# wkh923/m3pc

Measured on AMD Instinct MI355X. Metric: MPC plan-steps/sec (N=1024, H=16, hopper-medium-v2); independent plan steps, 3 in flight, higher is better.
Workload: dtype bf16; 1 GPU; hopper-medium-v2 shapes (S=11,A=3) rtg_guiding N=1024 H=16 T=32 bf16 candidate pass + fp32 policy pass + fp32 re-score (arg-max and multinomial draw certified under the calibrated bound delta, 8.4 candidates re-scored on average); 3 independent plan steps in flight (policy pass / candidate pass / re-score of neighbouring steps on different streams); window resident in HBM; candidates_per_gpu=1024, global_candidates=1024, horizon=16, traj_length=32, steps_in_flight=3, settle_steps=24, parallelism=1 GPU

## Files before the change

include/m3pc_hip_debug.h:

```cpp
#ifndef M3PC_HIP_DEBUG_H
#define M3PC_HIP_DEBUG_H

#ifdef __cplusplus
extern "C" {
#endif

int m3pc_debug_gemm(int dtype, const void* A, const void* Wt, const float* bias, const float* res, void* C, int M, int N,
                    int K, int gelu, int f32out, int variant, void* stream);
typedef struct m3pc_debug_gemm_args {
    int dtype;
    const void* A;
    int lda;
    int amap[3];
    const void* W;
    int ldw;
    int M, N, K;
    const float* bias;
    const float* rowtab;
    int rt_mod, rt_ld;
    int gelu;
    const float* res;
    int ldr;
    void* C;
    int f32out;
    int ldc;
    int cmap[3];
    float* ws;
    long long ws_bytes;
    int a_padded;
    const float* ln_g;
    const float* ln_b;
    float* ln_out;
    const float* a_ln_g;
    const float* a_ln_b;
    int variant;
    void* stream;
    int* picked;
} m3pc_debug_gemm_args;
int m3pc_debug_gemm_ex(const m3pc_debug_gemm_args* a);
int m3pc_debug_gemm_plan(const m3pc_debug_gemm_args* a);
int m3pc_debug_gemm_group(const m3pc_debug_gemm_args* a, int n);
int m3pc_debug_clock(long long* out2);
int m3pc_debug_clock_big(long long* out4);
int m3pc_debug_topk(const float* v, int n, int k, int* idx_out, void* stream);
int m3pc_debug_calibrate_stats(const float* scores_low, const float* f32, int n, float factor, float* stats, float* delta_out,
                               void* stream);
int m3pc_debug_topk_race_batch(const float* scores, const float* expo, float temperature, int n_windows, int n_total, int kmax, int kmin,
                               int rmax, int* list, float* list_scores, void* stream);
int m3pc_debug_gather_listed(const float* sample_actions, const int* list, int n_windows, int n_total, int row_floats, int list_stride,
                             int lo, int hi, float* cand, int* window_index, void* stream);
typedef struct m3pc_debug_tail_args {
    const float* scores;
    const float* expo;
    int race, select;
    float temperature;
    int n_windows, n_total;
    const int* list;
    const float* list_scores;
    const float* list_rescored;
    int rmax, list_stride, f_stride, f_lo;
    const int* r;
    const int* n;
    const float* delta;
    float* merged;
    float* stats;
    float* host_stats;
    float seq;
    const float* a0;
    long long a0_window_stride, a0_stride;
    int A;
    float* p;
    float* eval_action;
    int* argmax;
    int* sample_idx;
    float* sample_action;
    void* stream;
} m3pc_debug_tail_args;
int m3pc_debug_merge_select_batch(const m3pc_debug_tail_args* a);
int m3pc_debug_select_batch(const float* scores, const float* a0, long long a0_window_stride, long long a0_stride, int n_windows,
                            int n_total, int A, float temperature, const float* expo, float* p, float* eval_action, int* argmax,
                            int* sample_idx, float* sample_action, void* stream);
typedef struct m3pc_debug_eval_batch_args {
    const float* merged;
    int n_windows, n_total;
    const int* list;
    int rmax, list_stride, n_listed;
    const int* r;
    const int* n;
// ... 147 lines not shown
```

m3pc_amd/build.py:

```python
from __future__ import annotations

import os
import subprocess
import sys
from concurrent.futures import ThreadPoolExecutor

HERE = os.path.dirname(os.path.abspath(__file__))
CSRC = os.path.join(HERE, "csrc")
LIB = os.path.join(HERE, "libm3pc_hip.so")
SOURCES = ["gemm.hip", "gemm_x3.hip", "gemm_glds.hip", "gemm_big.hip", "gemm_line.hip", "gemm_f32_direct.hip", "block_fused.hip", "attn.hip",
           "attn_bf16.hip", "elementwise.hip", "select.hip", "refine.hip", "m3pc_plans.hip", "m3pc_passes.hip", "m3pc.hip", "m3pc_certified.hip"]
LAB_SOURCES = ["gemm_ring.hip", "gemm_persist.hip", "gemm_rs.hip", "m3pc_debug.hip"]
LAB_LIB = os.path.join(HERE, "libm3pc_hip_lab.so")
ARCH = "gfx950"
EXTRA_FLAGS = {"block_fused.hip": ["-fno-slp-vectorize"]}


def _hipcc() -> str:
    for c in (os.environ.get("HIPCC"), "/opt/rocm/bin/hipcc", "hipcc"):
        if c and (os.path.isabs(c) and os.path.exists(c) or not os.path.isabs(c)):
            return c
    raise RuntimeError("hipcc not found")


def _stale(target: str, deps) -> bool:
    if not os.path.exists(target):
        return True
    t = os.path.getmtime(target)
    return any(os.path.getmtime(d) > t for d in deps)


def build_library(force: bool = False, verbose: bool = False, lab: bool = False) -> str:
    hipcc = _hipcc()
    headers = [os.path.join(CSRC, n) for n in ("kernels.h", "gemm_epilogue.h", "gemm_stage_asm.h", "m3pc_internal.h", "cert_resolve.h", "exports.map")] + \
              [os.path.join(os.path.dirname(HERE), "include", n) for n in ("m3pc_hip.h", "m3pc_hip_debug.h")]
    objdir = os.path.join(CSRC, "build_lab" if lab else "build")
    os.makedirs(objdir, exist_ok=True)
    flags = ["-O3", f"--offload-arch={ARCH}", "-fPIC", "-std=c++17", "-Wall", "-Wno-unused-function",
             "-fno-gpu-rdc", "-ffp-contract=off", "-fvisibility=hidden"] + (["-DM3PC_LAB"] if lab else [])
    jobs = []
    objs = []
    lib = LAB_LIB if lab else LIB
    for s in SOURCES + (LAB_SOURCES if lab else []):
        src = os.path.join(CSRC, s)
        obj = os.path.join(objdir, s.replace(".hip", ".o"))
        objs.append(obj)
        if force or _stale(obj, [src] + headers):
            jobs.append([hipcc, *flags, *EXTRA_FLAGS.get(s, []), "-c", src, "-o", obj])

    def run(cmd):
        if verbose:
            print(" ".join(cmd), flush=True)
        r = subprocess.run(cmd, capture_output=True, text=True)
        if r.returncode != 0:
            raise RuntimeError("hipcc failed:\n" + " ".join(cmd) + "\n" + r.stdout + r.stderr)
        if verbose and r.stderr.strip():
            print(r.stderr)

    with ThreadPoolExecutor(max_workers=4) as ex:
        list(ex.map(run, jobs))
    if force or jobs or _stale(lib, objs):
        run([hipcc, "-shared", "-fPIC", f"--offload-arch={ARCH}", f"-Wl,--version-script={os.path.join(CSRC, 'exports.map')}", "-o", lib, *objs])
    return lib


if __name__ == "__main__":
    print(build_library(force="--force" in sys.argv, verbose=True, lab="--lab" in sys.argv))
```

m3pc_amd/csrc/gemm.hip:

```cpp
#include "kernels.h"

namespace m3pc {

#ifdef M3PC_LAB
thread_local int g_gemm_picked[4] = {0, 0, 0, 0};
thread_local int g_gemm_dry = 0;
#endif

typedef float f32x16 __attribute__((ext_vector_type(16)));
typedef float f32x4 __attribute__((ext_vector_type(4)));
typedef __bf16 bf16x8 __attribute__((ext_vector_type(8)));
typedef unsigned int u32x4 __attribute__((ext_vector_type(4)));

#define LDS_ROW 144

enum { EPI_GELU = 1, EPI_RES = 2, EPI_ROWTAB = 4, EPI_F32OUT = 8, EPI_SPLITK = 16 };

__device__ __forceinline__ float gelu_exact(float x) { return 0.5f * x * (1.0f + erff(x * 0.70710678118654752440f)); }
__device__ __forceinline__ float gelu_fast(float x) {
    const float ax = fabsf(x) * 0.70710678118654752440f;
    const float t = __builtin_amdgcn_rcpf(fmaf(0.3275911f, ax, 1.0f));
    float p = fmaf(t, 1.061405429f, -1.453152027f);
    p = fmaf(t, p, 1.421413741f);
    p = fmaf(t, p, -0.284496736f);
    p = fmaf(t, p, 0.254829592f);
    p *= t;
    const float e = __builtin_amdgcn_exp2f(-ax * ax * 1.44269504088896340736f);
    const float erf_abs = fmaf(-p, e, 1.0f);
    const float hx = 0.5f * x;
    return fmaf(fabsf(hx), erf_abs, hx);
}

__device__ __forceinline__ int map_row(const RowMap& m, int r) {
    if (m.rpg == 0) return r;
    return (r / m.rpg) * m.gstride + (r % m.rpg) + m.off;
}

template <typename T, int BM, int BN, int EPI>
__global__ __launch_bounds__(256) void gemm_kernel(GemmP p) {
    constexpr int TM = BM / 64, TN = BN / 64;
    constexpr int A_CH = BM * 8 / 256, W_CH = BN * 8 / 256;
    constexpr int BUF = (BM + BN) * LDS_ROW;
    __shared__ __attribute__((aligned(16))) char smem[2 * BUF];

    const int tid = threadIdx.x;
    const int lane = tid & 63, wid = tid >> 6;
    const int wr = wid >> 1, wc = wid & 1;
    const int ntn = p.N / BN;
    const int ntm = (p.M + BM - 1) / BM;
    const int nwg = ntm * ntn;
    int bid = blockIdx.x;
    {
        const int q = nwg / 8, r = nwg % 8, x = bid % 8, i = bid / 8;
        bid = (x < r ? x * (q + 1) : r * (q + 1) + (x - r) * q) + i;
    }
    const int tm = bid / ntn, tn = bid % ntn;
    const int row0 = tm * BM, col0 = tn * BN;

    const char* Ab = (const char*)p.A;
    const char* Wb = (const char*)p.W;
    const long long lda_b = (long long)p.lda * sizeof(T), ldw_b = (long long)p.ldw * sizeof(T);
    const int nkt = (int)((long long)p.K * sizeof(T) / 128);
    int kt0 = 0, kt1 = nkt;
    if constexpr (EPI & EPI_SPLITK) {
        kt0 = (int)((long long)nkt * blockIdx.y / gridDim.y);
        kt1 = (int)((long long)nkt * (blockIdx.y + 1) / gridDim.y);
    }

    const char* a_src[A_CH];
    int a_dst[A_CH];
#pragma unroll
    for (int i = 0; i < A_CH; ++i) {
        const int c = tid + i * 256, r = c >> 3, kc = c & 7;
        int gr = row0 + r;
        if (gr >= p.M) gr = p.M - 1;
        a_src[i] = Ab + (long long)map_row(p.amap, gr) * lda_b + kc * 16 + (long long)kt0 * 128;
        a_dst[i] = r * LDS_ROW + kc * 16;
    }
    const char* w_src[W_CH];
    int w_dst[W_CH];
#pragma unroll
    for (int i = 0; i < W_CH; ++i) {
        const int c = tid + i * 256, r = c >> 3, kc = c & 7;
        w_src[i] = Wb + (long long)(col0 + r) * ldw_b + kc * 16 + (long long)kt0 * 128;
        w_dst[i] = BM * LDS_ROW + r * LDS_ROW + kc * 16;
    }

    f32x16 acc[TM][TN];
#pragma unroll
    for (int i = 0; i < TM; ++i)
#pragma unroll
        for (int j = 0; j < TN; ++j)
#pragma unroll
            for (int e = 0; e < 16; ++e) acc[i][j][e] = 0.f;

    const int nloc = kt1 - kt0;
    u32x4 ra0[A_CH], rw0[W_CH], ra1[A_CH], rw1[W_CH];
    auto gload = [&](u32x4* ra, u32x4* rw, int kt) {
        const long long ko = (long long)kt * 128;
#pragma unroll
        for (int i = 0; i < A_CH; ++i) ra[i] = *(const u32x4*)(a_src[i] + ko);
#pragma unroll
        for (int i = 0; i < W_CH; ++i) rw[i] = *(const u32x4*)(w_src[i] + ko);
    };
    auto lstore = [&](const u32x4* ra, const u32x4* rw, char* buf) {
#pragma unroll
        for (int i = 0; i < A_CH; ++i) *(u32x4*)(buf + a_dst[i]) = ra[i];
#pragma unroll
        for (int i = 0; i < W_CH; ++i) *(u32x4*)(buf + w_dst[i]) = rw[i];
    };
    gload(ra0, rw0, 0);
    lstore(ra0, rw0, smem);
    if (nloc > 1) gload(ra0, rw0, 1);
    if (nloc > 2) gload(ra1, rw1, 2);
    __syncthreads();

    const int fragA = (wr * (BM / 2) + (lane & 31)) * LDS_ROW + 16 * (lane >> 5);
    const int fragW = BM * LDS_ROW + (wc * (BN / 2) + (lane & 31)) * LDS_ROW + 16 * (lane >> 5);

    auto compute = [&](const char* cur) {
#pragma unroll
        for (int s = 0; s < 4; ++s) {
            u32x4 fa[TM], fw[TN];
#pragma unroll
            for (int i = 0; i < TM; ++i) fa[i] = *(const u32x4*)(cur + fragA + i * 32 * LDS_ROW + 32 * s);
#pragma unroll
            for (int j = 0; j < TN; ++j) fw[j] = *(const u32x4*)(cur + fragW + j * 32 * LDS_ROW + 32 * s);
#pragma unroll
            for (int i = 0; i < TM; ++i)
#pragma unroll
                for (int j = 0; j < TN; ++j) {
                    if constexpr (sizeof(T) == 2) {
                        acc[i][j] = __builtin_amdgcn_mfma_f32_32x32x16_bf16(
                            __builtin_bit_cast(bf16x8, fa[i]), __builtin_bit_cast(bf16x8, fw[j]), acc[i][j], 0, 0, 0);
                    } else {
                        const f32x4 a4 = __builtin_bit_cast(f32x4, fa[i]);
                        const f32x4 w4 = __builtin_bit_cast(f32x4, fw[j]);
#pragma unroll
                        for (int e = 0; e < 4; ++e)
                            acc[i][j] = __builtin_amdgcn_mfma_f32_32x32x2f32(a4[e], w4[e], acc[i][j], 0, 0, 0);
                    }
                }
        }
    };
    auto step = [&](u32x4* ra, u32x4* rw, int kt) {
        compute(smem + (kt & 1) * BUF);
        if (kt + 1 < nloc) lstore(ra, rw, smem + ((kt + 1) & 1) * BUF);
        __syncthreads();
        if (kt + 3 < nloc) gload(ra, rw, kt + 3);
    };
    for (int kt = 0; kt < nloc; kt += 2) {
        step(ra0, rw0, kt);
        if (kt + 1 < nloc) step(ra1, rw1, kt + 1);
    }

    if constexpr (EPI & EPI_SPLITK) {
        float* slab = p.ws + (long long)blockIdx.y * p.M * p.N;
#pragma unroll
        for (int i = 0; i < TM; ++i)
#pragma unroll
            for (int reg = 0; reg < 16; ++reg) {
                const int r = row0 + wr * (BM / 2) + i * 32 + (reg & 3) + 8 * (reg >> 2) + 4 * (lane >> 5);
                if (r < p.M) {
#pragma unroll
                    for (int j = 0; j < TN; ++j)
                        slab[(long long)r * p.N + col0 + wc * (BN / 2) + j * 32 + (lane & 31)] = acc[i][j][reg];
                }
            }
        return;
    }
    float bj[TN];
#pragma unroll
    for (int j = 0; j < TN; ++j) bj[j] = p.bias ? p.bias[col0 + wc * (BN / 2) + j * 32 + (lane & 31)] : 0.f;
#pragma unroll
    for (int i = 0; i < TM; ++i) {
#pragma unroll
        for (int reg = 0; reg < 16; ++reg) {
            const int r = row0 + wr * (BM / 2) + i * 32 + (reg & 3) + 8 * (reg >> 2) + 4 * (lane >> 5);
            if (r < p.M) {
                const long long pr = map_row(p.cmap, r);
#pragma unroll
                for (int j = 0; j < TN; ++j) {
                    const int c = col0 + wc * (BN / 2) + j * 32 + (lane & 31);
                    float v = acc[i][j][reg] + bj[j];
                    if constexpr (EPI & EPI_ROWTAB) v += p.rowtab[(long long)(r % p.rt_mod) * p.rt_ld + c];
                    if constexpr (EPI & EPI_GELU) v = sizeof(T) == 2 ? gelu_fast(v) : gelu_exact(v);
                    if constexpr (EPI & EPI_RES) v += p.res[pr * p.ldr + c];
                    if constexpr ((EPI & EPI_F32OUT) || sizeof(T) == 4)
                        p.Cf[pr * p.ldc + c] = v;
                    else
                        p.Cb[pr * p.ldc + c] = (bf16_t)v;
                }
            }
        }
    }
}

__global__ __launch_bounds__(256) void splitk_reduce_kernel(GemmP p, int S, int exact_gelu) {
    const long long n = (long long)p.M * p.N;
    for (long long x = blockIdx.x * 256LL + threadIdx.x; x < n; x += (long long)gridDim.x * 256) {
        const int r = (int)(x / p.N), c = (int)(x % p.N);
        float v = 0.f;
        for (int s = 0; s < S; ++s) v += p.ws[(long long)s * n + x];
        if (p.bias) v += p.bias[c];
        if (p.rowtab) v += p.rowtab[(long long)(r % p.rt_mod) * p.rt_ld + c];
        if (p.gelu) v = exact_gelu ? gelu_exact(v) : gelu_fast(v);
        const long long pr = map_row(p.cmap, r);
        if (p.res) v += p.res[pr * p.ldr + c];
        if (p.Cf) p.Cf[pr * p.ldc + c] = v;
        if (p.Cb) p.Cb[pr * p.ldc + c] = (bf16_t)v;
// ... 32 lines not shown
            for (; k < S; ++k) a += *(const f32x4r*)(src + k * mn);
#pragma unroll
            for (int e = 0; e < 4; ++e) {
                float x = a[e];
                if (p.bias) x += p.bias[c + e];
                if (p.rowtab) x += p.rowtab[(long long)(r % p.rt_mod) * p.rt_ld + c + e];
                if (p.gelu) x = exact_gelu ? gelu_exact(x) : gelu_fast(x);
                if (p.res) x += p.res[(long long)r * p.ldr + c + e];
                a[e] = x;
            }
            *(f32x4r*)(p.Cf + (long long)r * p.ldc + c) = a;
            v[i] = a;
            s += (a[0] + a[1]) + (a[2] + a[3]);
        }
    const float inv_d = 1.0f / (float)p.N;
    const float mean = wave_sum_r(s) * inv_d;
    float q = 0.f;
#pragma unroll
    for (int i = 0; i < 4; ++i)
        if (i < n) {
#pragma unroll
            for (int e = 0; e < 4; ++e) {
                const float c = v[i][e] - mean;
                q += c * c;
            }
        }
    const float rstd = rsqrtf(wave_sum_r(q) * inv_d + 1e-5f);
#pragma unroll
    for (int i = 0; i < 4; ++i)
        if (i < n) {
            const int c = i * 256 + lane * 4;
            const f32x4r g = *(const f32x4r*)(p.ln_g + c);
            const f32x4r b = *(const f32x4r*)(p.ln_b + c);
            f32x4r y;
#pragma unroll
            for (int e = 0; e < 4; ++e) y[e] = (v[i][e] - mean) * rstd * g[e] + b[e];
            *(f32x4r*)(p.ln_out + (long long)r * p.N + c) = y;
        }
}

int launch_splitk_reduce(const GemmP& p, int S, int exact_gelu, hipStream_t st) {
    if (p.ln_g && p.ln_out && p.Cf && !p.Cb && p.cmap.rpg == 0 && p.N % 256 == 0 && p.N <= 1024 && p.ldc % 4 == 0 &&
        (!p.res || p.ldr % 4 == 0)) {
        M3PC_GEMM_LAUNCH(splitk_reduce_ln_kernel, dim3((p.M + 3) / 4), dim3(256), 0, st, p, S, exact_gelu);
        M3PC_GEMM_PICK_FLAG(2);
        return 1;
    }
    const long long n = (long long)p.M * p.N;
    const int g = (int)((n + 255) / 256 < 1024 ? (n + 255) / 256 : 1024);
    M3PC_GEMM_LAUNCH(splitk_reduce_kernel, dim3(g), dim3(256), 0, st, p, S, exact_gelu);
    return 0;
}

template <typename T, int BM, int BN, int EPI>
static void launch_cfg(const GemmP& p, hipStream_t st) {
    const int grid = ((p.M + BM - 1) / BM) * (p.N / BN);
    M3PC_GEMM_LAUNCH((gemm_kernel<T, BM, BN, EPI>), dim3(grid), dim3(256), 0, st, p);
}

template <typename T, int EPI>
static int launch_epi(const GemmP& p, hipStream_t st) {
    const long long big_tiles = (long long)((p.M + 127) / 128) * (p.N / 128);
    if ((p.N % 128) != 0 || big_tiles < 512) {
        const long long tiles = (long long)((p.M + 63) / 64) * (p.N / 64);
        const int nkt = (int)((long long)p.K * sizeof(T) / 128);
        int S = 1;
        if (sizeof(T) == 4 && p.ws && tiles < 768 && (tiles < 200 || nkt > 16)) {
            S = (int)((1023 + tiles) / tiles);
            if (S > nkt / 4) S = nkt / 4;
            if (S > 16) S = 16;
            while (S > 1 && (long long)S * p.M * p.N * 4 > p.ws_bytes) --S;
        }
        M3PC_GEMM_PICK(sizeof(T) == 4 ? 1 : 3, S, 0, 0);
        if (S > 1) {
            M3PC_GEMM_LAUNCH((gemm_kernel<T, 64, 64, EPI_SPLITK>), dim3((unsigned)tiles, S), dim3(256), 0, st, p);
            return launch_splitk_reduce(p, S, (int)(sizeof(T) == 4), st);
        } else {
            launch_cfg<T, 64, 64, EPI>(p, st);
        }
    } else {
        M3PC_GEMM_PICK(sizeof(T) == 4 ? 2 : 4, 1, 0, 0);
        launch_cfg<T, 128, 128, EPI>(p, st);
    }
    return 0;
}

template <typename T>
static int launch_t(const GemmP& p, hipStream_t st) {
    const bool f32out = sizeof(T) == 4 || p.Cf != nullptr;
    const int epi = (p.gelu ? EPI_GELU : 0) | (p.res ? EPI_RES : 0) | (p.rowtab ? EPI_ROWTAB : 0) |
                    (f32out && sizeof(T) == 2 ? EPI_F32OUT : 0);
    switch (epi) {
        case 0: return launch_epi<T, 0>(p, st);
        case EPI_F32OUT: return launch_epi<T, EPI_F32OUT>(p, st);
        case EPI_GELU: return launch_epi<T, EPI_GELU>(p, st);
        case EPI_GELU | EPI_F32OUT: return launch_epi<T, EPI_GELU | EPI_F32OUT>(p, st);
        case EPI_RES: return launch_epi<T, EPI_RES>(p, st);
        case EPI_RES | EPI_F32OUT: return launch_epi<T, EPI_RES | EPI_F32OUT>(p, st);
        case EPI_ROWTAB: return launch_epi<T, EPI_ROWTAB>(p, st);
        case EPI_ROWTAB | EPI_F32OUT: return launch_epi<T, EPI_ROWTAB | EPI_F32OUT>(p, st);
        default: M3PC_GEMM_PICK(0, 0, 0, 0); return 0;
    }
}

int launch_gemm(const GemmP& p, int dtype, hipStream_t st) {
    if (p.M <= 0) return 0;
#ifdef M3PC_LAB
    if (dtype == DT_BF16 && p.variant == 9 && launch_gemm_persist(p, st)) return 0;
    if (dtype == DT_BF16 && p.variant == 36 && launch_gemm_rs(p, st)) return 0;
#endif
    static const bool no_big = M3PC_ENV("M3PC_NO_GEMM_BIG") != nullptr;
    if (dtype == DT_BF16 && p.variant >= 37 && p.variant <= 42 && launch_gemm_big(p, st)) return 0;
    if (dtype == DT_BF16 && p.variant >= 43 && p.variant <= 46 && launch_gemm_line(p, p.variant == 44 ? 256 : 128, st)) return 0;
    static const bool no_line = M3PC_ENV("M3PC_NO_GEMM_LINE") != nullptr;
    static const long long line_min = M3PC_ENV("M3PC_LINE_MIN_TILES") ? atoll(M3PC_ENV("M3PC_LINE_MIN_TILES")) : 256;
    if (dtype == DT_BF16 && p.variant == 0 && !no_line && !p.res && p.K < 1024 &&
        (long long)((p.M + 127) / 128) * (p.N / 128) >= line_min && launch_gemm_line(p, 128, st))
        return 0;
    if (dtype == DT_BF16 && p.variant == 0 && !no_big && p.K >= 1024 && (long long)((p.M + 255) / 256) * (p.N / 256) >= 224 &&
        launch_gemm_big(p, st))
        return 0;
#ifdef M3PC_LAB
    if (dtype == DT_BF16 && p.variant >= 7 && p.variant != 9 && p.variant < 20 && launch_gemm_ring(p, st)) return 0;
#endif
    if (dtype == DT_BF16 && (p.variant == 0 || (p.variant >= 2 && p.variant < 7) || (p.variant >= 20 && p.variant <= 32)) &&
        launch_gemm_glds(p, st))
        return 0;
    if (dtype == DT_BF16) return launch_t<bf16_t>(p, st);
    static const bool no_direct = M3PC_ENV("M3PC_NO_F32_DIRECT") != nullptr;
    if (p.ws && p.variant != 2 && !no_direct && launch_gemm_f32_direct(p, st)) return 0;
    return launch_t<float>(p, st);
}

}
```

m3pc_amd/csrc/gemm_x3.hip:

```cpp
#include "gemm_epilogue.h"

namespace m3pc {

typedef float x3_f32x16 __attribute__((ext_vector_type(16)));
typedef float x3_f32x4 __attribute__((ext_vector_type(4)));
typedef __bf16 x3_bf16x8 __attribute__((ext_vector_type(8)));
typedef __bf16 x3_bf16x4 __attribute__((ext_vector_type(4)));
typedef unsigned int x3_u32x4 __attribute__((ext_vector_type(4)));
typedef unsigned int x3_u32x2 __attribute__((ext_vector_type(2)));

#define X3_ROW 144
enum { X3_SPLITK = 1 << 8 };

__device__ __forceinline__ void x3_split4(x3_u32x4 raw, x3_u32x2& hi, x3_u32x2& lo) {
    const x3_f32x4 x = __builtin_bit_cast(x3_f32x4, raw);
    x3_bf16x4 h, l;
#pragma unroll
    for (int e = 0; e < 4; ++e) {
        h[e] = (__bf16)x[e];
        l[e] = (__bf16)(x[e] - (float)h[e]);
    }
    hi = __builtin_bit_cast(x3_u32x2, h);
    lo = __builtin_bit_cast(x3_u32x2, l);
}

__device__ __forceinline__ int x3_map_row(const RowMap& m, int r) {
    if (m.rpg == 0) return r;
    return (r / m.rpg) * m.gstride + (r % m.rpg) + m.off;
}

template <int BM, int BN, int EPI>
__global__ __launch_bounds__(256) void gemm_x3_kernel(GemmP p) {
    constexpr int TM = BM / 64, TN = BN / 64;
    constexpr int A_CH = BM * 8 / 256, W_CH = BN * 8 / 256;
    constexpr int BUF = (BM + BN) * X3_ROW;
    __shared__ __attribute__((aligned(16))) char smem[2 * BUF];

    const int tid = threadIdx.x;
    const int lane = tid & 63, wid = tid >> 6;
    const int wr = wid >> 1, wc = wid & 1;
    const int ntn = p.N / BN;
    const int ntm = (p.M + BM - 1) / BM;
    const int nwg = ntm * ntn;
    int bid = blockIdx.x;
    {
        const int q = nwg / 8, r = nwg % 8, x = bid % 8, i = bid / 8;
        bid = (x < r ? x * (q + 1) : r * (q + 1) + (x - r) * q) + i;
    }
    const int tm = bid / ntn, tn = bid % ntn;
    const int row0 = tm * BM, col0 = tn * BN;

    const char* Ab = (const char*)p.A;
    const char* Wb = (const char*)p.W;
    const long long lda_b = (long long)p.lda * 4, ldw_b = (long long)p.ldw * 2, wlo_b = p.w_lo_off * 2;
    const int nkt = p.K / 32;
    int kt0 = 0, kt1 = nkt;
    if constexpr (EPI & X3_SPLITK) {
        kt0 = (int)((long long)nkt * blockIdx.y / gridDim.y);
        kt1 = (int)((long long)nkt * (blockIdx.y + 1) / gridDim.y);
    }

    const char* a_src[A_CH];
    int a_dst[A_CH];
#pragma unroll
    for (int i = 0; i < A_CH; ++i) {
        const int c = tid + i * 256, r = c >> 3, kc = c & 7;
        int gr = row0 + r;
        if (gr >= p.M) gr = p.M - 1;
        a_src[i] = Ab + (long long)x3_map_row(p.amap, gr) * lda_b + kc * 16 + (long long)kt0 * 128;
        a_dst[i] = r * X3_ROW + kc * 8;
    }
    const char* w_src[W_CH];
    int w_dst[W_CH];
#pragma unroll
    for (int i = 0; i < W_CH; ++i) {
        const int c = tid + i * 256, r = c >> 3, kc = c & 7;
        w_src[i] = Wb + (long long)(col0 + r) * ldw_b + (kc & 3) * 16 + (kc >> 2) * wlo_b + (long long)kt0 * 64;
        w_dst[i] = BM * X3_ROW + r * X3_ROW + kc * 16;
    }

    x3_f32x16 acc[TM][TN];
#pragma unroll
    for (int i = 0; i < TM; ++i)
#pragma unroll
        for (int j = 0; j < TN; ++j)
#pragma unroll
            for (int e = 0; e < 16; ++e) acc[i][j][e] = 0.f;

    const int nloc = kt1 - kt0;
    x3_u32x4 ra0[A_CH], rw0[W_CH], ra1[A_CH], rw1[W_CH];
    auto gload = [&](x3_u32x4* ra, x3_u32x4* rw, int kt) {
#pragma unroll
        for (int i = 0; i < A_CH; ++i) ra[i] = *(const x3_u32x4*)(a_src[i] + (long long)kt * 128);
#pragma unroll
        for (int i = 0; i < W_CH; ++i) rw[i] = *(const x3_u32x4*)(w_src[i] + (long long)kt * 64);
    };
    auto lstore = [&](const x3_u32x4* ra, const x3_u32x4* rw, char* buf) {
#pragma unroll
        for (int i = 0; i < A_CH; ++i) {
            x3_u32x2 hi, lo;
            x3_split4(ra[i], hi, lo);
            *(x3_u32x2*)(buf + a_dst[i]) = hi;
            *(x3_u32x2*)(buf + a_dst[i] + 64) = lo;
        }
#pragma unroll
        for (int i = 0; i < W_CH; ++i) *(x3_u32x4*)(buf + w_dst[i]) = rw[i];
    };
    gload(ra0, rw0, 0);
    lstore(ra0, rw0, smem);
    if (nloc > 1) gload(ra0, rw0, 1);
    if (nloc > 2) gload(ra1, rw1, 2);
    __syncthreads();

    const int fragA = (wr * (BM / 2) + (lane & 31)) * X3_ROW + 16 * (lane >> 5);
    const int fragW = BM * X3_ROW + (wc * (BN / 2) + (lane & 31)) * X3_ROW + 16 * (lane >> 5);

    auto compute = [&](const char* cur) {
#pragma unroll
        for (int s = 0; s < 2; ++s) {
            x3_u32x4 ah[TM], al[TM], wh[TN], wl[TN];
#pragma unroll
            for (int i = 0; i < TM; ++i) {
                ah[i] = *(const x3_u32x4*)(cur + fragA + i * 32 * X3_ROW + 32 * s);
                al[i] = *(const x3_u32x4*)(cur + fragA + i * 32 * X3_ROW + 64 + 32 * s);
            }
#pragma unroll
            for (int j = 0; j < TN; ++j) {
                wh[j] = *(const x3_u32x4*)(cur + fragW + j * 32 * X3_ROW + 32 * s);
                wl[j] = *(const x3_u32x4*)(cur + fragW + j * 32 * X3_ROW + 64 + 32 * s);
            }
#pragma unroll
            for (int i = 0; i < TM; ++i)
#pragma unroll
                for (int j = 0; j < TN; ++j) {
                    const x3_bf16x8 a_h = __builtin_bit_cast(x3_bf16x8, ah[i]), a_l = __builtin_bit_cast(x3_bf16x8, al[i]);
                    const x3_bf16x8 w_h = __builtin_bit_cast(x3_bf16x8, wh[j]), w_l = __builtin_bit_cast(x3_bf16x8, wl[j]);
                    acc[i][j] = __builtin_amdgcn_mfma_f32_32x32x16_bf16(a_h, w_h, acc[i][j], 0, 0, 0);
                    acc[i][j] = __builtin_amdgcn_mfma_f32_32x32x16_bf16(a_h, w_l, acc[i][j], 0, 0, 0);
                    acc[i][j] = __builtin_amdgcn_mfma_f32_32x32x16_bf16(a_l, w_h, acc[i][j], 0, 0, 0);
                }
        }
    };
    auto step = [&](x3_u32x4* ra, x3_u32x4* rw, int kt) {
        compute(smem + (kt & 1) * BUF);
        if (kt + 1 < nloc) lstore(ra, rw, smem + ((kt + 1) & 1) * BUF);
        __syncthreads();
        if (kt + 3 < nloc) gload(ra, rw, kt + 3);
    };
    for (int kt = 0; kt < nloc; kt += 2) {
        step(ra0, rw0, kt);
        if (kt + 1 < nloc) step(ra1, rw1, kt + 1);
    }

    if constexpr (EPI & X3_SPLITK) {
        float* slab = p.ws + (long long)blockIdx.y * p.M * p.N;
#pragma unroll
        for (int i = 0; i < TM; ++i)
#pragma unroll
            for (int reg = 0; reg < 16; ++reg) {
                const int r = row0 + wr * (BM / 2) + i * 32 + (reg & 3) + 8 * (reg >> 2) + 4 * (lane >> 5);
                if (r < p.M) {
#pragma unroll
                    for (int j = 0; j < TN; ++j)
                        slab[(long long)r * p.N + col0 + wc * (BN / 2) + j * 32 + (lane & 31)] = acc[i][j][reg];
                }
            }
        return;
    } else {
        const int wu = __builtin_amdgcn_readfirstlane(wid);
        const int rbase = row0 + (wu >> 1) * (BM / 2), cbase = col0 + (wu & 1) * (BN / 2);
        gemm_epilogue<EPI, TM, TN>(p, acc, rbase, cbase, row0, BM, lane);
    }
}

__global__ __launch_bounds__(256) void f32_split_bf16_kernel(const float* in, bf16_t* hi, bf16_t* lo, long long n) {
    for (long long x = blockIdx.x * 256LL + threadIdx.x; x < n; x += (long long)gridDim.x * 256) {
        const float v = in[x];
        const bf16_t b = (bf16_t)v;
        hi[x] = b;
        lo[x] = (bf16_t)(v - (float)b);
    }
}
void launch_f32_split_bf16(const float* in, bf16_t* hi, bf16_t* lo, long long n, hipStream_t st) {
    if (n <= 0) return;
    const long long g = (n + 255) / 256;
    hipLaunchKernelGGL(f32_split_bf16_kernel, dim3((unsigned)(g < 4096 ? g : 4096)), dim3(256), 0, st, in, hi, lo, n);
}

template <int BM, int BN, int EPI>
static void x3_launch(const GemmP& p, int S, hipStream_t st) {
    const int grid = ((p.M + BM - 1) / BM) * (p.N / BN);
    M3PC_GEMM_LAUNCH((gemm_x3_kernel<BM, BN, EPI>), dim3(grid, S), dim3(256), 0, st, p);
}

template <int EPI>
static int x3_launch_epi(const GemmP& p, hipStream_t st) {
    const long long big_tiles = (long long)((p.M + 127) / 128) * (p.N / 128);
    if ((p.N % 128) == 0 && big_tiles >= 512) {
        M3PC_GEMM_PICK(13, 1, 0, 0);
        x3_launch<128, 128, EPI>(p, 1, st);
        return 0;
    }
    const long long tiles = (long long)((p.M + 63) / 64) * (p.N / 64);
    const int nkt = p.K / 32;
    int S = 1;
    if (p.ws && tiles < 768 && (tiles < 200 || nkt > 16)) {
        S = (int)((1023 + tiles) / tiles);
        if (S > nkt / 4) S = nkt / 4;
        if (S > 16) S = 16;
        while (S > 1 && (long long)S * p.M * p.N * 4 > p.ws_bytes) --S;
    }
    M3PC_GEMM_PICK(12, S, 0, 0);
    if (S > 1) {
        x3_launch<64, 64, X3_SPLITK>(p, S, st);
        return launch_splitk_reduce(p, S, 1, st);
    }
    x3_launch<64, 64, EPI>(p, 1, st);
    return 0;
}

int launch_gemm_x3(const GemmP& p, hipStream_t st) {
    if (p.M <= 0) return 0;
    if (p.K % 32 != 0 || p.N % 64 != 0 || p.w_lo_off <= 0 || p.w_lo_off % 8 != 0 || (p.Cf == nullptr) == (p.Cb == nullptr)) return -1;
    if (((uintptr_t)p.A & 15) || ((uintptr_t)p.W & 15) || p.lda % 4 != 0 || p.ldw % 8 != 0 || p.a_ln_g) return -1;
    const int epi = (p.gelu ? GE_GELU | GE_GELU_EXACT : 0) | (p.res ? GE_RES : 0) | (p.rowtab ? GE_ROWTAB : 0) |
                    (p.Cf ? GE_F32OUT : 0);
    switch (epi) {
        case GE_F32OUT: return x3_launch_epi<GE_F32OUT>(p, st);
        case GE_GELU | GE_GELU_EXACT | GE_F32OUT: return x3_launch_epi<GE_GELU | GE_GELU_EXACT | GE_F32OUT>(p, st);
        case GE_RES | GE_F32OUT: return x3_launch_epi<GE_RES | GE_F32OUT>(p, st);
        case GE_ROWTAB | GE_F32OUT: return x3_launch_epi<GE_ROWTAB | GE_F32OUT>(p, st);
        case 0: return x3_launch_epi<0>(p, st);
        case GE_GELU | GE_GELU_EXACT: return x3_launch_epi<GE_GELU | GE_GELU_EXACT>(p, st);
        default: return -1;
    }
}

}
```

m3pc_amd/csrc/kernels.h:

```cpp
#pragma once
#include <hip/hip_runtime.h>
#include <stdint.h>

#ifdef M3PC_LAB
#define M3PC_ENV(name) getenv(name)
#else
#define M3PC_ENV(name) ((const char*)nullptr)
#endif

namespace m3pc {

typedef __bf16 bf16_t;

enum DType { DT_F32 = 0, DT_BF16 = 1, DT_X3 = 2 };

static inline size_t dtype_size(int dt) { return dt == DT_F32 ? 4 : 2; }

#ifndef M3PC_STREAM_AUX
#define M3PC_STREAM_AUX 0
#endif
template <typename V>
__device__ __forceinline__ V stream_load(const V* p) { return M3PC_STREAM_AUX ? __builtin_nontemporal_load(p) : *p; }
template <typename V>
__device__ __forceinline__ void stream_store(V v, V* p) {
    if (M3PC_STREAM_AUX) __builtin_nontemporal_store(v, p);
    else *p = v;
}

struct RowMap {
    int rpg;
    int gstride;
    int off;
};
static inline RowMap rowmap_identity() { return RowMap{0, 0, 0}; }

struct GemmP {
    const void* A;
    int lda;
    RowMap amap;
    const void* W;
    int ldw;
    int M, N, K;
    const float* bias;
    const float* rowtab;
    int rt_mod, rt_ld;
    int gelu;
    const float* res;
    int ldr;
    float* Cf;
    bf16_t* Cb;
    int ldc;
    RowMap cmap;
    float* ws;
    long long ws_bytes;
    int a_padded;
    int variant;
    int peel;
    const float* ln_g;
    const float* ln_b;
    float* ln_out;
    const float* a_ln_g;
    const float* a_ln_b;
    long long w_lo_off;
};
struct HeadFusedP {
    const float* X;
    int ldx;
    int rows, d;
    int n_heads;
    int grp, row_mod;
    const float *gA, *bA;
    const float *gB[2], *bB[2];
    const float *W1[2], *b1[2];
    const float *w2[2], *b2[2];
    const float *mean[2], *stdv[2];
    float* out[2];
    float* part;
    int* ticket;
};
bool launch_head_f32_fused(const HeadFusedP& p, hipStream_t st);
int launch_gemm(const GemmP& p, int dtype, hipStream_t st);
int launch_gemm_x3(const GemmP& p, hipStream_t st);
void launch_f32_split_bf16(const float* in, bf16_t* hi, bf16_t* lo, long long n, hipStream_t st);
int launch_splitk_reduce(const GemmP& p, int S, int exact_gelu, hipStream_t st);
bool gemm_f32_direct_covers(const GemmP& p);
bool launch_gemm_f32_direct_group(const GemmP* ps, int n, hipStream_t st);
bool launch_gemm_ring(const GemmP& p, hipStream_t st);
bool launch_gemm_persist(const GemmP& p, hipStream_t st);
bool launch_gemm_rs(const GemmP& p, hipStream_t st);
bool launch_gemm_big(const GemmP& p, hipStream_t st);
bool launch_gemm_line(const GemmP& p, int bt, hipStream_t st);
bool launch_gemm_glds(const GemmP& p, hipStream_t st);
void read_big_probe(long long out[4]);
void read_clock_probe(long long out[2]);
bool launch_gemm_f32_direct(const GemmP& p, hipStream_t st);

__host__ __device__ inline int block_res_row_xb(int r, int L, int nshared) {
    const int b = r / L, w = r % L;
    return w < nshared ? w : nshared + b * (L - nshared) + (w - nshared);
}

struct BlockP {
    const bf16_t* O;
    int ldo;
    int M;
    const float* res;
    int ldr;
    int res_L, res_nshared;
    const float* rowtab;
    int rt_mod;
    int res_nu;
    const bf16_t* wstream;
    const float* bo;
    const float* b1;
    const float* b2;
    const float* ln2_g;
    const float* ln2_b;
    float* Xout;
    int ldx;
    int x_bf16;
    const float* lnA_g;
    const float* lnA_b;
    const float* lnB_g[2];
    const float* lnB_b[2];
    int out_mod, out_grp;
    bf16_t* Hout;
    int ldh;
    bf16_t* QKVout;
    int ldq;
    unsigned qkv_bytes;
    const float* bqkv;
    float* head_out[2];
    const float* hb1[2];
    const float* hw2[2];
    const float* hb2[2];
    const float* hmean[2];
    const float* hstd[2];
    int split;
    int variant;
    long long* stamps;
    int stamp_block;
};
bool block_fused_supported(int d, int ff);
size_t block_stream_bytes();
void launch_pack_block_stream(const bf16_t* Wo, const bf16_t* W1, const bf16_t* W2, bf16_t* out, hipStream_t st);
void launch_pack_block_qkv(const bf16_t* Wqkv_next, bf16_t* out, hipStream_t st);
void launch_pack_block_heads(const bf16_t* Wh0, const bf16_t* Wh1, bf16_t* out, hipStream_t st);
bool launch_block_fused(const BlockP& p, hipStream_t st);
// ... 349 lines not shown
```

m3pc_amd/csrc/m3pc_debug.hip:

```cpp
#include "m3pc_internal.h"

#pragma GCC visibility push(default)
extern "C" {

int m3pc_debug_step_streams_created(m3pc_handle* h) { return h ? h->step_streams_created : -1; }
int m3pc_debug_gemm(int dtype, const void* A, const void* Wt, const float* bias, const float* res, void* C, int M, int N,
                    int K, int gelu, int f32out, int variant, void* stream) {
    static const int ldpad = M3PC_ENV("M3PC_DEBUG_LDPAD") ? atoi(M3PC_ENV("M3PC_DEBUG_LDPAD")) : 0;
    GemmP p = gemm_basic(A, K + ldpad, Wt, K + ldpad, M, N, K, bias);
    p.a_padded = 0;
    p.gelu = gelu;
    p.res = res;
    p.ldr = N;
    p.variant = variant;
    if (dtype == DT_BF16 && !f32out)
        p.Cb = (bf16_t*)C;
    else
        p.Cf = (float*)C;
    p.ldc = N;
    if (dtype != DT_BF16 && variant != 1) {
        static float* ws = nullptr;
        if (!ws) HIPCHK(hipMalloc((void**)&ws, 64 << 20));
        p.ws = ws;
        p.ws_bytes = 64 << 20;
    }
    if (dtype == DT_X3) {
        static bf16_t* wsplit = nullptr;
        static size_t cap = 0;
        const size_t n = (size_t)N * (K + ldpad);
        if (n > cap) {
            if (wsplit) HIPCHK(hipFree(wsplit));
            wsplit = nullptr;
            cap = 0;
            HIPCHK(hipMalloc((void**)&wsplit, 2 * n * sizeof(bf16_t)));
            cap = n;
        }
        launch_f32_split_bf16((const float*)Wt, wsplit, wsplit + n, (long long)n, (hipStream_t)stream);
        p.W = wsplit;
        p.w_lo_off = (long long)n;
        if (launch_gemm_x3(p, (hipStream_t)stream) < 0) return fail(M3PC_EINVAL, "debug_gemm: shape not covered by the x3 kernel");
        return check_launch("debug_gemm");
    }
    launch_gemm(p, dtype, (hipStream_t)stream);
    return check_launch("debug_gemm");
}

static int debug_gemm_fill(const m3pc_debug_gemm_args* a, GemmP& p) {
    if (!a) return fail(M3PC_EINVAL, "debug_gemm_ex: null argument");
    const int dt = a->dtype;
    if (dt != DT_F32 && dt != DT_BF16 && dt != DT_X3) return fail(M3PC_EINVAL, "debug_gemm_ex: dtype %d", dt);
    if (!a->A || !a->W || !a->C) return fail(M3PC_EINVAL, "debug_gemm_ex: null operand");
    if (a->M < 1 || a->M > (1 << 20) || a->N < 32 || a->N > (1 << 16) || a->K < 1 || a->K > (1 << 16)) return fail(M3PC_EINVAL, "debug_gemm_ex: M / N / K out of range");
    const int es = dt == DT_BF16 ? 2 : 4;
    if (a->N % 32) return fail(M3PC_EINVAL, "debug_gemm_ex: N %d is not a multiple of 32 (columns would be dropped)", a->N);
    if (((long long)a->K * es) % 128) return fail(M3PC_EINVAL, "debug_gemm_ex: K %d is not a whole number of 128-byte k-tiles (k terms would be dropped)", a->K);
    if (dt == DT_F32 && !a->f32out) return fail(M3PC_EINVAL, "debug_gemm_ex: fp32 operands have fp32 output only");
    const int f32out = dt == DT_F32 || a->f32out;
    const int os = f32out ? 4 : 2;
    const uintptr_t ptrs = (uintptr_t)a->A | (uintptr_t)a->W | (uintptr_t)a->C | (uintptr_t)a->bias | (uintptr_t)a->rowtab | (uintptr_t)a->res |
                           (uintptr_t)a->ws | (uintptr_t)a->ln_g | (uintptr_t)a->ln_b | (uintptr_t)a->ln_out | (uintptr_t)a->a_ln_g |
                           (uintptr_t)a->a_ln_b;
    if (ptrs & 15) return fail(M3PC_EINVAL, "debug_gemm_ex: pointers must be 16-byte aligned");
    if (a->lda < a->K || a->ldw < a->K || a->ldc < a->N || (a->res && a->ldr < a->N) || (a->rowtab && a->rt_ld < a->N))
        return fail(M3PC_EINVAL, "debug_gemm_ex: a leading dimension is below its row length");
    if (((long long)a->lda * es) % 16 || ((long long)a->ldw * (dt == DT_F32 ? 4 : 2)) % 16 || (dt == DT_X3 && a->ldw % 4) || ((long long)a->ldc * os) % 16 ||
        (a->res && a->ldr % 4) || (a->rowtab && a->rt_ld % 4))
        return fail(M3PC_EINVAL, "debug_gemm_ex: rows of a leading dimension leave 16-byte alignment");
    if (a->rowtab && a->rt_mod < 1) return fail(M3PC_EINVAL, "debug_gemm_ex: rowtab with rt_mod %d", a->rt_mod);
    for (const int* m : {a->amap, a->cmap})
        if (m[0] < 0 || m[2] < 0 || (m[0] >= 1 && m[1] < m[0])) return fail(M3PC_EINVAL, "debug_gemm_ex: row map {%d, %d, %d}", m[0], m[1], m[2]);
    if (a->ws && a->ws_bytes < 0) return fail(M3PC_EINVAL, "debug_gemm_ex: negative ws_bytes");
    if (a->ln_out && (!f32out || !a->ln_g || !a->ln_b)) return fail(M3PC_EINVAL, "debug_gemm_ex: ln_out needs fp32 C, ln_g and ln_b");
    if ((a->a_ln_g != nullptr) != (a->a_ln_b != nullptr)) return fail(M3PC_EINVAL, "debug_gemm_ex: a_ln_g and a_ln_b go together");
    const int v = a->variant;
    if (!(v == 0 || (dt == DT_BF16 && (v == 2 || v == 26 || v == 37 || v == 43 || v == 44)) || (dt == DT_F32 && v == 2)))
        return fail(M3PC_EINVAL, "debug_gemm_ex: variant %d of dtype %d is not one this hook drives", v, dt);
    if (v == 44 && a->a_padded && a->M % 256 && 256 - a->M % 256 > 127)
        return fail(M3PC_EINVAL, "debug_gemm_ex: variant 44 with a_padded would read %d rows behind A", 256 - a->M % 256);
    p = gemm_basic(a->A, a->lda, a->W, a->ldw, a->M, a->N, a->K, a->bias);
    p.amap = RowMap{a->amap[0], a->amap[1], a->amap[2]};
    p.cmap = RowMap{a->cmap[0], a->cmap[1], a->cmap[2]};
    p.rowtab = a->rowtab;
    if (a->rowtab) {
        p.rt_mod = a->rt_mod;
        p.rt_ld = a->rt_ld;
    }
    p.gelu = a->gelu ? 1 : 0;
    p.res = a->res;
    p.ldr = a->ldr;
    if (f32out)
        p.Cf = (float*)a->C;
    else
        p.Cb = (bf16_t*)a->C;
    p.ldc = a->ldc;
    p.ws = a->ws;
    p.ws_bytes = a->ws ? a->ws_bytes : 0;
    p.a_padded = a->a_padded ? 1 : 0;
    p.ln_g = a->ln_out ? a->ln_g : nullptr;
    p.ln_b = a->ln_out ? a->ln_b : nullptr;
    p.ln_out = a->ln_out;
    p.a_ln_g = a->a_ln_g;
    p.a_ln_b = a->a_ln_b;
    p.variant = v;
    if (a->a_ln_g && (dt != DT_F32 || !a->ws || v == 2 || !gemm_f32_direct_covers(p)))
        return fail(M3PC_EINVAL, "debug_gemm_ex: a_ln_* on a problem the few-row fp32 kernel does not take (the fold would be dropped)");
    return 0;
}

static int debug_gemm_plan(const m3pc_debug_gemm_args* a, GemmP& p, int* plan) {
    if (a && a->picked) a->picked[0] = a->picked[1] = a->picked[2] = a->picked[3] = 0;
    if (int rc = debug_gemm_fill(a, p)) return rc;
    const int dt = a->dtype;
    if (dt == DT_X3) p.w_lo_off = (long long)a->N * a->ldw;
    M3PC_GEMM_PICK(0, 0, 0, 0);
    g_gemm_dry = 1;
    const int dry = dt == DT_X3 ? launch_gemm_x3(p, nullptr) : launch_gemm(p, dt, nullptr);
    g_gemm_dry = 0;
    for (int i = 0; i < 4; ++i) plan[i] = g_gemm_picked[i];
    if (dry < 0 || plan[0] == 0) return fail(M3PC_EINVAL, "debug_gemm_ex: no kernel of the dispatch covers this problem (epilogue flags / shape)");
    if (a->N % 64 && plan[0] != 5)
        return fail(M3PC_EINVAL, "debug_gemm_ex: N %d is not a multiple of 64 (kernel %d would drop columns)", a->N, plan[0]);
    const int v = a->variant;
    const int want = dt != DT_BF16 ? 0 : v == 2 ? 8 : v == 26 ? 7 : v == 37 ? 9 : v == 43 ? 10 : v == 44 ? 11 : 0;
    if (want && plan[0] != want) return fail(M3PC_EINVAL, "debug_gemm_ex: variant %d does not take this problem (kernel %d would run)", v, plan[0]);
    return 0;
}

int m3pc_debug_gemm_plan(const m3pc_debug_gemm_args* a) {
    GemmP p;
    int plan[4];
    if (int rc = debug_gemm_plan(a, p, plan)) return rc;
    if (a->picked)
        for (int i = 0; i < 4; ++i) a->picked[i] = plan[i];
    return 0;
}

int m3pc_debug_gemm_ex(const m3pc_debug_gemm_args* a) {
    GemmP p;
    int plan[4];
    if (int rc = debug_gemm_plan(a, p, plan)) return rc;
    hipStream_t st = (hipStream_t)a->stream;
    if (a->dtype == DT_X3) {
        static bf16_t* wsplit = nullptr;
        static size_t cap = 0;
        const size_t nw = (size_t)a->N * a->ldw;
        if (nw > cap) {
            if (wsplit) HIPCHK(hipFree(wsplit));
            wsplit = nullptr;
            cap = 0;
            HIPCHK(hipMalloc((void**)&wsplit, 2 * nw * sizeof(bf16_t)));
            cap = nw;
        }
        launch_f32_split_bf16((const float*)a->W, wsplit, wsplit + nw, (long long)nw, st);
        p.W = wsplit;
    }
    M3PC_GEMM_PICK(0, 0, 0, 0);
// ... 756 lines not shown
```

Measured before the change: 874.2 plan-steps/s.

## Choose GEMM workgroup tile order by modeled per-XCD operand traffic

Adds a host-side model that estimates the bytes each of the 8 contiguous workgroup runs (one per XCD) must load under row-panel, column-panel or k-slice orderings, and picks the cheapest. The kernels map blockIdx through the chosen order, and split-K now also remaps the k-slice index so slices can be interleaved across XCDs. The aim is to cut duplicated A/W fetches across XCD L2 caches. It costs extra index arithmetic in every kernel and a small host-side loop per launch, and an env var can force an order.

```diff
diff --git a/include/m3pc_hip_debug.h b/include/m3pc_hip_debug.h
--- a/include/m3pc_hip_debug.h
+++ b/include/m3pc_hip_debug.h
@@ -34,6 +34,7 @@
     const float* a_ln_g;
     const float* a_ln_b;
     int variant;
+    int order;
     void* stream;
     int* picked;
 } m3pc_debug_gemm_args;
diff --git a/m3pc_amd/build.py b/m3pc_amd/build.py
--- a/m3pc_amd/build.py
+++ b/m3pc_amd/build.py
@@ -32,7 +32,7 @@
 
 def build_library(force: bool = False, verbose: bool = False, lab: bool = False) -> str:
     hipcc = _hipcc()
-    headers = [os.path.join(CSRC, n) for n in ("kernels.h", "gemm_epilogue.h", "gemm_stage_asm.h", "m3pc_internal.h", "cert_resolve.h", "exports.map")] + \
+    headers = [os.path.join(CSRC, n) for n in ("kernels.h", "gemm_order.h", "gemm_epilogue.h", "gemm_stage_asm.h", "m3pc_internal.h", "cert_resolve.h", "exports.map")] + \
               [os.path.join(os.path.dirname(HERE), "include", n) for n in ("m3pc_hip.h", "m3pc_hip_debug.h")]
     objdir = os.path.join(CSRC, "build_lab" if lab else "build")
     os.makedirs(objdir, exist_ok=True)
diff --git a/m3pc_amd/csrc/gemm.hip b/m3pc_amd/csrc/gemm.hip
--- a/m3pc_amd/csrc/gemm.hip
+++ b/m3pc_amd/csrc/gemm.hip
@@ -1,3 +1,5 @@
+#include <cstring>
+
 #include "kernels.h"
 
 namespace m3pc {
@@ -48,14 +50,8 @@
     const int wr = wid >> 1, wc = wid & 1;
     const int ntn = p.N / BN;
     const int ntm = (p.M + BM - 1) / BM;
-    const int nwg = ntm * ntn;
-    int bid = blockIdx.x;
-    {
-        const int q = nwg / 8, r = nwg % 8, x = bid % 8, i = bid / 8;
-        bid = (x < r ? x * (q + 1) : r * (q + 1) + (x - r) * q) + i;
-    }
-    const int tm = bid / ntn, tn = bid % ntn;
-    const int row0 = tm * BM, col0 = tn * BN;
+    const GemmBlock blk = gemm_block_of(p.order, (int)(blockIdx.x + gridDim.x * blockIdx.y), ntm, ntn, (int)gridDim.y);
+    const int row0 = blk.tm * BM, col0 = blk.tn * BN;
 
     const char* Ab = (const char*)p.A;
     const char* Wb = (const char*)p.W;
@@ -63,8 +59,8 @@
     const int nkt = (int)((long long)p.K * sizeof(T) / 128);
     int kt0 = 0, kt1 = nkt;
     if constexpr (EPI & EPI_SPLITK) {
-        kt0 = (int)((long long)nkt * blockIdx.y / gridDim.y);
-        kt1 = (int)((long long)nkt * (blockIdx.y + 1) / gridDim.y);
+        kt0 = (int)((long long)nkt * blk.ks / gridDim.y);
+        kt1 = (int)((long long)nkt * (blk.ks + 1) / gridDim.y);
     }
 
     const char* a_src[A_CH];
@@ -155,7 +151,7 @@
     }
 
     if constexpr (EPI & EPI_SPLITK) {
-        float* slab = p.ws + (long long)blockIdx.y * p.M * p.N;
+        float* slab = p.ws + (long long)blk.ks * p.M * p.N;
 #pragma unroll
         for (int i = 0; i < TM; ++i)
 #pragma unroll
@@ -294,35 +290,39 @@
     return 0;
 }
 
+int gemm_order_forced() {
+    static const int forced = [] {
+        const char* e = M3PC_ENV("M3PC_GEMM_ORDER");
+        if (!e) return (int)GEMM_ORDER_AUTO;
+        return !strcmp(e, "row") ? (int)GEMM_ROW_PANEL : !strcmp(e, "col") ? (int)GEMM_COL_PANEL : !strcmp(e, "kslice") ? (int)GEMM_K_SLICE : (int)GEMM_ORDER_AUTO;
+    }();
+    return forced;
+}
+
 template <typename T, int BM, int BN, int EPI>
-static void launch_cfg(const GemmP& p, hipStream_t st) {
+static void launch_cfg(const GemmP& p_in, int S, hipStream_t st) {
+    GemmP p = p_in;
+    const int nkt = (int)((long long)p.K * sizeof(T) / 128);
+    p.order = gemm_order_pick(p.order ? p.order : gemm_order_forced(), p.M, p.N, nkt, S, BM, BN);
     const int grid = ((p.M + BM - 1) / BM) * (p.N / BN);
-    M3PC_GEMM_LAUNCH((gemm_kernel<T, BM, BN, EPI>), dim3(grid), dim3(256), 0, st, p);
+    M3PC_GEMM_LAUNCH((gemm_kernel<T, BM, BN, EPI>), dim3(grid, S), dim3(256), 0, st, p);
 }
 
 template <typename T, int EPI>
 static int launch_epi(const GemmP& p, hipStream_t st) {
-    const long long big_tiles = (long long)((p.M + 127) / 128) * (p.N / 128);
-    if ((p.N % 128) != 0 || big_tiles < 512) {
-        const long long tiles = (long long)((p.M + 63) / 64) * (p.N / 64);
+    if (!gemm_takes_big_tiles(p.M, p.N)) {
         const int nkt = (int)((long long)p.K * sizeof(T) / 128);
-        int S = 1;
-        if (sizeof(T) == 4 && p.ws && tiles < 768 && (tiles < 200 || nkt > 16)) {
-            S = (int)((1023 + tiles) / tiles);
-            if (S > nkt / 4) S = nkt / 4;
-            if (S > 16) S = 16;
-            while (S > 1 && (long long)S * p.M * p.N * 4 > p.ws_bytes) --S;
-        }
+        const int S = sizeof(T) == 4 && p.ws ? gemm_split_count(p.M, p.N, nkt, p.ws_bytes) : 1;
         M3PC_GEMM_PICK(sizeof(T) == 4 ? 1 : 3, S, 0, 0);
         if (S > 1) {
-            M3PC_GEMM_LAUNCH((gemm_kernel<T, 64, 64, EPI_SPLITK>), dim3((unsigned)tiles, S), dim3(256), 0, st, p);
+            launch_cfg<T, 64, 64, EPI_SPLITK>(p, S, st);
             return launch_splitk_reduce(p, S, (int)(sizeof(T) == 4), st);
         } else {
-            launch_cfg<T, 64, 64, EPI>(p, st);
+            launch_cfg<T, 64, 64, EPI>(p, 1, st);
         }
     } else {
         M3PC_GEMM_PICK(sizeof(T) == 4 ? 2 : 4, 1, 0, 0);
-        launch_cfg<T, 128, 128, EPI>(p, st);
+        launch_cfg<T, 128, 128, EPI>(p, 1, st);
     }
     return 0;
 }
diff --git a/m3pc_amd/csrc/gemm_order.h b/m3pc_amd/csrc/gemm_order.h
--- /dev/null
+++ b/m3pc_amd/csrc/gemm_order.h
@@ -0,0 +1,111 @@
+#pragma once
+
+#if defined(__HIPCC__)
+#define M3PC_ORDER_HD __host__ __device__
+#else
+#define M3PC_ORDER_HD
+#endif
+
+namespace m3pc {
+
+enum GemmOrder { GEMM_ORDER_AUTO = 0, GEMM_ROW_PANEL = 1, GEMM_COL_PANEL = 2, GEMM_K_SLICE = 3 };
+
+struct GemmBlock {
+    int tm, tn, ks;
+};
+
+M3PC_ORDER_HD inline int gemm_run_start(int x, int n) {
+    const int q = n / 8, r = n % 8;
+    return x < r ? x * (q + 1) : r * (q + 1) + (x - r) * q;
+}
+M3PC_ORDER_HD inline int gemm_run_item(int b, int n) { return gemm_run_start(b % 8, n) + b / 8; }
+
+M3PC_ORDER_HD inline GemmBlock gemm_block_of(int order, int lin, int ntm, int ntn, int S) {
+    const int nwg = ntm * ntn;
+    GemmBlock g;
+    if (order == GEMM_K_SLICE) {
+        const int it = gemm_run_item(lin, nwg * S);
+        const int t = it % nwg;
+        g.ks = it / nwg;
+        g.tm = t / ntn;
+        g.tn = t % ntn;
+    } else {
+        const int t = gemm_run_item(lin % nwg, nwg);
+        g.ks = lin / nwg;
+        if (order == GEMM_COL_PANEL) {
+            g.tn = t / ntm;
+            g.tm = t % ntm;
+        } else {
+            g.tm = t / ntn;
+            g.tn = t % ntn;
+        }
+    }
+    return g;
+}
+
+
+inline bool gemm_takes_big_tiles(int M, int N) { return N % 128 == 0 && (long long)((M + 127) / 128) * (N / 128) >= 512; }
+
+inline int gemm_split_count(int M, int N, int nkt, long long ws_bytes) {
+    const long long tiles = (long long)((M + 63) / 64) * (N / 64);
+    int S = 1;
+    if (tiles < 768 && (tiles < 200 || nkt > 16)) {
+        S = (int)((1023 + tiles) / tiles);
+        if (S > nkt / 4) S = nkt / 4;
+        if (S > 16) S = 16;
+        while (S > 1 && (long long)S * M * N * 4 > ws_bytes) --S;
+    }
+    return S;
+}
+
+inline long long gemm_panel_rows(int first, int len, int ntm, int M, int BM) {
+    if (len >= ntm) return M;
+    long long rows = (long long)len * BM;
+    if (first + len - 1 >= ntm - 1) rows -= (long long)ntm * BM - M;
+    return rows;
+}
+inline long long gemm_run_rows(int order, int a, int b, int ntm, int ntn, int M, int BM, int BN) {
+    if (b <= a) return 0;
+    const int len = b - a;
+    if (order == GEMM_COL_PANEL) {
+        const int cols = (b - 1) / ntm - a / ntm + 1;
+        return gemm_panel_rows(a % ntm, len, ntm, M, BM) + (long long)cols * BN;
+    }
+    const int p0 = a / ntn, p1 = (b - 1) / ntn;
+    const long long end = (long long)(p1 + 1) * BM < M ? (long long)(p1 + 1) * BM : M;
+    return end - (long long)p0 * BM + (long long)(len < ntn ? len : ntn) * BN;
+}
+
+inline long long gemm_order_bytes(int order, int M, int N, int nkt, int S, int BM, int BN) {
+    const int ntm = (M + BM - 1) / BM, ntn = N / BN, nwg = ntm * ntn;
+    long long bytes = 0;
+    for (int x = 0; x < 8; ++x) {
+        if (order != GEMM_K_SLICE || S <= 1) {
+            bytes += gemm_run_rows(order == GEMM_COL_PANEL ? order : GEMM_ROW_PANEL, gemm_run_start(x, nwg), gemm_run_start(x + 1, nwg), ntm,
+                                   ntn, M, BM, BN) * nkt * 128;
+            continue;
+        }
+        const int a = gemm_run_start(x, nwg * S), b = gemm_run_start(x + 1, nwg * S);
+        for (int ks = a / nwg; ks * nwg < b; ++ks) {
+            const int lo = a > ks * nwg ? a - ks * nwg : 0, hi = b < (ks + 1) * nwg ? b - ks * nwg : nwg;
+            const int kt = (int)((long long)nkt * (ks + 1) / S) - (int)((long long)nkt * ks / S);
+            bytes += gemm_run_rows(GEMM_ROW_PANEL, lo, hi, ntm, ntn, M, BM, BN) * kt * 128;
+        }
+    }
+    return bytes;
+}
+
+inline int gemm_order_choose(int M, int N, int nkt, int S, int BM, int BN) {
+    int best = GEMM_ROW_PANEL;
+    long long bb = gemm_order_bytes(GEMM_ROW_PANEL, M, N, nkt, S, BM, BN);
+    const long long bc = gemm_order_bytes(GEMM_COL_PANEL, M, N, nkt, S, BM, BN);
+    if (bc < bb) best = GEMM_COL_PANEL, bb = bc;
+    if (S > 1 && gemm_order_bytes(GEMM_K_SLICE, M, N, nkt, S, BM, BN) < bb) best = GEMM_K_SLICE;
+    return best;
+}
+inline int gemm_order_pick(int forced, int M, int N, int nkt, int S, int BM, int BN) {
+    const int o = forced >= GEMM_ROW_PANEL && forced <= GEMM_K_SLICE ? forced : gemm_order_choose(M, N, nkt, S, BM, BN);
+    return o == GEMM_K_SLICE && S <= 1 ? GEMM_ROW_PANEL : o;
+}
+
+}
diff --git a/m3pc_amd/csrc/gemm_x3.hip b/m3pc_amd/csrc/gemm_x3.hip
--- a/m3pc_amd/csrc/gemm_x3.hip
+++ b/m3pc_amd/csrc/gemm_x3.hip
@@ -41,14 +41,8 @@
     const int wr = wid >> 1, wc = wid & 1;
     const int ntn = p.N / BN;
     const int ntm = (p.M + BM - 1) / BM;
-    const int nwg = ntm * ntn;
-    int bid = blockIdx.x;
-    {
-        const int q = nwg / 8, r = nwg % 8, x = bid % 8, i = bid / 8;
-        bid = (x < r ? x * (q + 1) : r * (q + 1) + (x - r) * q) + i;
-    }
-    const int tm = bid / ntn, tn = bid % ntn;
-    const int row0 = tm * BM, col0 = tn * BN;
+    const GemmBlock blk = gemm_block_of(p.order, (int)(blockIdx.x + gridDim.x * blockIdx.y), ntm, ntn, (int)gridDim.y);
+    const int row0 = blk.tm * BM, col0 = blk.tn * BN;
 
     const char* Ab = (const char*)p.A;
     const char* Wb = (const char*)p.W;
@@ -56,8 +50,8 @@
     const int nkt = p.K / 32;
     int kt0 = 0, kt1 = nkt;
     if constexpr (EPI & X3_SPLITK) {
-        kt0 = (int)((long long)nkt * blockIdx.y / gridDim.y);
-        kt1 = (int)((long long)nkt * (blockIdx.y + 1) / gridDim.y);
+        kt0 = (int)((long long)nkt * blk.ks / gridDim.y);
+        kt1 = (int)((long long)nkt * (blk.ks + 1) / gridDim.y);
     }
 
     const char* a_src[A_CH];
@@ -153,7 +147,7 @@
     }
 
     if constexpr (EPI & X3_SPLITK) {
-        float* slab = p.ws + (long long)blockIdx.y * p.M * p.N;
+        float* slab = p.ws + (long long)blk.ks * p.M * p.N;
 #pragma unroll
         for (int i = 0; i < TM; ++i)
 #pragma unroll
@@ -188,28 +182,21 @@
 }
 
 template <int BM, int BN, int EPI>
-static void x3_launch(const GemmP& p, int S, hipStream_t st) {
+static void x3_launch(const GemmP& p_in, int S, hipStream_t st) {
+    GemmP p = p_in;
+    p.order = gemm_order_pick(p.order ? p.order : gemm_order_forced(), p.M, p.N, p.K / 32, S, BM, BN);
     const int grid = ((p.M + BM - 1) / BM) * (p.N / BN);
     M3PC_GEMM_LAUNCH((gemm_x3_kernel<BM, BN, EPI>), dim3(grid, S), dim3(256), 0, st, p);
 }
 
 template <int EPI>
 static int x3_launch_epi(const GemmP& p, hipStream_t st) {
-    const long long big_tiles = (long long)((p.M + 127) / 128) * (p.N / 128);
-    if ((p.N % 128) == 0 && big_tiles >= 512) {
+    if (gemm_takes_big_tiles(p.M, p.N)) {
         M3PC_GEMM_PICK(13, 1, 0, 0);
         x3_launch<128, 128, EPI>(p, 1, st);
         return 0;
     }
-    const long long tiles = (long long)((p.M + 63) / 64) * (p.N / 64);
-    const int nkt = p.K / 32;
-    int S = 1;
-    if (p.ws && tiles < 768 && (tiles < 200 || nkt > 16)) {
-        S = (int)((1023 + tiles) / tiles);
-        if (S > nkt / 4) S = nkt / 4;
-        if (S > 16) S = 16;
-        while (S > 1 && (long long)S * p.M * p.N * 4 > p.ws_bytes) --S;
-    }
+    const int S = p.ws ? gemm_split_count(p.M, p.N, p.K / 32, p.ws_bytes) : 1;
     M3PC_GEMM_PICK(12, S, 0, 0);
     if (S > 1) {
         x3_launch<64, 64, X3_SPLITK>(p, S, st);
diff --git a/m3pc_amd/csrc/kernels.h b/m3pc_amd/csrc/kernels.h
--- a/m3pc_amd/csrc/kernels.h
+++ b/m3pc_amd/csrc/kernels.h
@@ -1,6 +1,8 @@
 #pragma once
 #include <hip/hip_runtime.h>
 #include <stdint.h>
+
+#include "gemm_order.h"
 
 #ifdef M3PC_LAB
 #define M3PC_ENV(name) getenv(name)
@@ -62,6 +64,7 @@
     const float* a_ln_g;
     const float* a_ln_b;
     long long w_lo_off;
+    int order;
 };
 struct HeadFusedP {
     const float* X;
@@ -94,6 +97,7 @@
 void read_big_probe(long long out[4]);
 void read_clock_probe(long long out[2]);
 bool launch_gemm_f32_direct(const GemmP& p, hipStream_t st);
+int gemm_order_forced();
 
 __host__ __device__ inline int block_res_row_xb(int r, int L, int nshared) {
     const int b = r / L, w = r % L;
diff --git a/m3pc_amd/csrc/m3pc_debug.hip b/m3pc_amd/csrc/m3pc_debug.hip
--- a/m3pc_amd/csrc/m3pc_debug.hip
+++ b/m3pc_amd/csrc/m3pc_debug.hip
@@ -75,6 +75,7 @@
     const int v = a->variant;
     if (!(v == 0 || (dt == DT_BF16 && (v == 2 || v == 26 || v == 37 || v == 43 || v == 44)) || (dt == DT_F32 && v == 2)))
         return fail(M3PC_EINVAL, "debug_gemm_ex: variant %d of dtype %d is not one this hook drives", v, dt);
+    if (a->order < GEMM_ORDER_AUTO || a->order > GEMM_K_SLICE) return fail(M3PC_EINVAL, "debug_gemm_ex: order %d (0 = the launcher's choice, 1 row panel, 2 column panel, 3 k-slice)", a->order);
     if (v == 44 && a->a_padded && a->M % 256 && 256 - a->M % 256 > 127)
         return fail(M3PC_EINVAL, "debug_gemm_ex: variant 44 with a_padded would read %d rows behind A", 256 - a->M % 256);
     p = gemm_basic(a->A, a->lda, a->W, a->ldw, a->M, a->N, a->K, a->bias);
@@ -102,6 +103,7 @@
     p.a_ln_g = a->a_ln_g;
     p.a_ln_b = a->a_ln_b;
     p.variant = v;
+    p.order = a->order;
     if (a->a_ln_g && (dt != DT_F32 || !a->ws || v == 2 || !gemm_f32_direct_covers(p)))
         return fail(M3PC_EINVAL, "debug_gemm_ex: a_ln_* on a problem the few-row fp32 kernel does not take (the fold would be dropped)");
     return 0;
```

New measurement: 874.5 plan-steps/s, median of 5. No clear change (+0.0%).
